# anonymousauthors001/SGS-GNN

Measured on AMD Instinct MI355X. Metric: sampled edges/sec + training steps/sec, Reddit hybrid 20% sparsity, higher is better.
Workload: dtype f32

## Files before the change

### sgs-gnn_amd/csrc/gcn.hip

```cpp
#include "sgs_common.h"

namespace sgs {
size_t graph_sort_workspace_bytes(int64_t n, int64_t N);
size_t graph_src_sorted_workspace_bytes(int64_t n, int64_t N);
int graph_build_src_sorted(const int64_t* ei, int64_t n, int64_t N, int32_t* in_ptr, int32_t* in_src, int32_t* in_eid, int32_t* out_ptr,
                           int32_t* out_dst, int32_t* out_eid, int32_t* loop_eid, int32_t* unsorted_flag, void* ws, size_t ws_bytes,
                           hipStream_t stream);
int graph_build_by_sort(const int64_t* ei, int64_t n, int64_t N, int32_t* in_ptr, int32_t* in_src, int32_t* in_eid, int32_t* out_ptr,
                        int32_t* out_dst, int32_t* out_eid, int32_t* loop_eid, void* ws, size_t ws_bytes, hipStream_t stream);
}

namespace sgs {
namespace {

constexpr int kT = 256;
constexpr int kMaxLdsRow = 8192;

__global__ void __launch_bounds__(kT) count_degrees(const int64_t* __restrict__ ei, int64_t n_edges, int* __restrict__ cnt_in,
                                                   int* __restrict__ cnt_out, int* __restrict__ loop_eid) {
    const int64_t e = static_cast<int64_t>(blockIdx.x) * kT + threadIdx.x;
    if (e >= n_edges) return;
    const int s = static_cast<int>(ei[e]), d = static_cast<int>(ei[n_edges + e]);
    atomicAdd(&cnt_in[d], 1);
    atomicAdd(&cnt_out[s], 1);
// ... 292 lines not shown
            cptr[row] = w;
            if (row == N - 1) cptr[N] = w + cnt[row];
        }
    } else {
        w = (out ? out_ptr : in_ptr)[row];
    }
    int loop = -1;
    const int b = pptr[row], e = pptr[row + 1];
    int pe_c = 0, col_c = 0;
    if (e > b) { const int kc = min(b + lane, e - 1); pe_c = peid[kc]; col_c = pcol[kc]; }
    for (int k0 = b; k0 < e; k0 += 64) {
        const int k = k0 + lane;
        const int kn = min(k + 64, e - 1);
        const int pe_n = peid[kn], col_n = pcol[kn];
        const bool m_c = mask_at<BITS>(mask, pe_c);
        const bool sel = k < e && m_c;
        const int ne = sel ? pos[pe_c] : 0;
        const int col = col_c;
        pe_c = pe_n; col_c = col_n;
        const unsigned long long bal = __ballot(sel);
        if (sel) {
            const int o = w + __popcll(bal & ((1ull << lane) - 1ull));
            ccol[o] = col;
            ceid[o] = ne;
        }
        if (!out) {
            const unsigned long long lb = __ballot(sel && col == static_cast<int>(row));
            if (lb) loop = __shfl(ne, 63 - __clzll(lb), 64);
        }
        w += __popcll(bal);
    }
    if (!out && lane == 0) loop_eid[row] = loop;
}
template <bool BITS, bool SCAN = false>
__global__ void __launch_bounds__(kT) filter_fill(const int* __restrict__ pin_ptr, const int* __restrict__ pin_src, const int* __restrict__ pin_eid,
                                                 const int* __restrict__ pout_ptr, const int* __restrict__ pout_dst,
                                                 const int* __restrict__ pout_eid, int64_t N, const uint8_t* __restrict__ mask,
                                                 const int* __restrict__ pos, int* __restrict__ in_ptr, int* __restrict__ in_src,
                                                 int* __restrict__ in_eid, int* __restrict__ out_ptr, int* __restrict__ out_dst,
                                                 int* __restrict__ out_eid, int* __restrict__ loop_eid, const int* __restrict__ cnt_in = nullptr,
                                                 const int* __restrict__ cnt_out = nullptr) {
    filter_fill_body<BITS, SCAN>(2 * N, pin_ptr, pin_src, pin_eid, pout_ptr, pout_dst, pout_eid, N, mask, pos, in_ptr, in_src, in_eid, out_ptr,
                                 out_dst, out_eid, loop_eid, cnt_in, cnt_out);
}

__device__ __forceinline__ void norm_deg_body(const float* __restrict__ w, int64_t N, const int* __restrict__ in_ptr,
                                              const int* __restrict__ in_src, const int* __restrict__ in_eid,
                                              const int* __restrict__ loop_eid, float* __restrict__ dis,
                                              float* __restrict__ loopw) {
    const int lane = threadIdx.x & 63;
    const int64_t i = (static_cast<int64_t>(blockIdx.x) * kT + threadIdx.x) >> 6;
    if (i >= N) return;
    const int b = in_ptr[i], e = in_ptr[i + 1];
    float acc = 0.f;
    for (int k = b + lane; k < e; k += 64) {
        if (in_src[k] != static_cast<int>(i)) acc += w ? w[in_eid[k]] : 1.0f;
    }
    acc = wave_sum_all(acc);
    const int le = loop_eid[i];
    const float lw = (le >= 0 && w) ? w[le] : 1.0f;
    const float deg = lw + acc;
    float di = 1.0f / sqrtf(deg);
    if (isinf(di)) di = 0.f;
    if (lane == 0) { dis[i] = di; loopw[i] = lw; }
}
__global__ void __launch_bounds__(kT) norm_deg(const float* __restrict__ w, int64_t N, const int* __restrict__ in_ptr,
                                              const int* __restrict__ in_src, const int* __restrict__ in_eid,
                                              const int* __restrict__ loop_eid, float* __restrict__ dis,
                                              float* __restrict__ loopw) {
    norm_deg_body(w, N, in_ptr, in_src, in_eid, loop_eid, dis, loopw);
}

__global__ void __launch_bounds__(kT) deg_partial(const float* __restrict__ w, int64_t N, const int* __restrict__ in_ptr,
                                                 const int* __restrict__ in_src, const int* __restrict__ in_eid,
                                                 float* __restrict__ degpart) {
    const int lane = threadIdx.x & 63;
    const int64_t i = (static_cast<int64_t>(blockIdx.x) * kT + threadIdx.x) >> 6;
    if (i >= N) return;
    float acc = 0.f;
    for (int k = in_ptr[i] + lane; k < in_ptr[i + 1]; k += 64)
        if (in_src[k] != static_cast<int>(i)) acc += w ? w[in_eid[k]] : 1.0f;
    acc = wave_sum_all(acc);
    if (lane == 0) degpart[i] = acc;
}
__global__ void __launch_bounds__(kT) dis_from_degree(const float* __restrict__ degsum, int64_t N, float* __restrict__ dis,
                                                     float* __restrict__ loopw) {
    const int64_t i = static_cast<int64_t>(blockIdx.x) * kT + threadIdx.x;
    if (i >= N) return;
    float di = 1.0f / sqrtf(1.0f + degsum[i]);
    if (isinf(di)) di = 0.f;
    dis[i] = di;
    loopw[i] = 1.0f;
}
__global__ void __launch_bounds__(kT) bias_act(const float* __restrict__ X, const float* __restrict__ bias, int64_t N, int64_t D, int act,
                                              float drop_scale, uint32_t drop_thresh, uint64_t seed, uint32_t site,
                                              const uint64_t* __restrict__ epoch, float* __restrict__ Y, int64_t row_offset) {
    seed = fold_epoch(seed, epoch);
    const int64_t idx = static_cast<int64_t>(blockIdx.x) * kT + threadIdx.x;
    if (idx >= N * D) return;
    const int64_t i = idx / D;
    const uint32_t c = static_cast<uint32_t>(idx - i * D);
    float y = X[idx];
    if (bias) y += bias[c];
    if (act != SGS_ACT_NONE) y = fmaxf(y, 0.f);
    if (act == SGS_ACT_RELU_DROPOUT) y = dropout_keep_at(seed, site, static_cast<uint64_t>(row_offset + i), c, drop_thresh) ? y * drop_scale : 0.f;
    Y[idx] = y;
}

__global__ void __launch_bounds__(kT) mean_weights(int64_t N, const int* __restrict__ in_ptr, const int* __restrict__ out_ptr,
                                                  const int* __restrict__ out_dst, float* __restrict__ what_in,
                                                  float* __restrict__ what_out) {
    const int lane = threadIdx.x & 63;
// ... 23 lines not shown
    logit[e] = prob * scale;
}

__device__ __forceinline__ void norm_weights_body(int64_t nrows, const float* __restrict__ w, int64_t N, int64_t n_edges,
                                                  const int* __restrict__ in_ptr, const int* __restrict__ in_src,
                                                  const int* __restrict__ in_eid, const int* __restrict__ out_ptr,
                                                  const int* __restrict__ out_dst, const int* __restrict__ out_eid,
                                                  const float* __restrict__ dis, const float* __restrict__ loopw,
                                                  float* __restrict__ what_in, float* __restrict__ what_out,
                                                  float* __restrict__ what_loop) {
    const int lane = threadIdx.x & 63;
    const int64_t r = (static_cast<int64_t>(blockIdx.x) * kT + threadIdx.x) >> 6;
    if (r >= nrows) return;
    const bool out = r >= N;
    const int i = static_cast<int>(out ? r - N : r);
    const float di = dis[i];
    if (!out) {
        const int b = in_ptr[i], e = in_ptr[i + 1];
        for (int k = b + lane; k < e; k += 64) {
            const int s = in_src[k];
            const float we = w ? w[in_eid[k]] : 1.0f;
            what_in[k] = (s == i) ? 0.f : (dis[s] * we) * di;
        }
        if (lane == 0) what_loop[i] = (di * loopw[i]) * di;
    } else {
        const int b = out_ptr[i], e = out_ptr[i + 1];
        for (int k = b + lane; k < e; k += 64) {
            const int t = out_dst[k];
            const float we = w ? w[out_eid[k]] : 1.0f;
            what_out[k] = (t == i) ? 0.f : (di * we) * dis[t];
        }
    }
}
__global__ void __launch_bounds__(kT) norm_weights(const float* __restrict__ w, int64_t N, int64_t n_edges,
                                                  const int* __restrict__ in_ptr, const int* __restrict__ in_src,
                                                  const int* __restrict__ in_eid, const int* __restrict__ out_ptr,
                                                  const int* __restrict__ out_dst, const int* __restrict__ out_eid,
                                                  const float* __restrict__ dis, const float* __restrict__ loopw,
                                                  float* __restrict__ what_in, float* __restrict__ what_out,
                                                  float* __restrict__ what_loop) {
    norm_weights_body(2 * N, w, N, n_edges, in_ptr, in_src, in_eid, out_ptr, out_dst, out_eid, dis, loopw, what_in, what_out, what_loop);
}

__global__ void __launch_bounds__(kT) norm_bwd_node(const float* __restrict__ w, const float* __restrict__ gw,
                                                   const float* __restrict__ gloop, int64_t N, const int* __restrict__ in_ptr,
                                                   const int* __restrict__ in_src, const int* __restrict__ in_eid,
                                                   const int* __restrict__ out_ptr, const int* __restrict__ out_dst,
                                                   const int* __restrict__ out_eid, const float* __restrict__ dis,
                                                   const float* __restrict__ loopw, float* __restrict__ Hn,
                                                   const float* __restrict__ gw2 = nullptr, const float* __restrict__ gloop2 = nullptr) {
    const int lane = threadIdx.x & 63;
    const int64_t t = (static_cast<int64_t>(blockIdx.x) * kT + threadIdx.x) >> 6;
    if (t >= N) return;
    float acc = 0.f;
    auto side = [&](const int* __restrict__ ptr, const int* __restrict__ col, const int* __restrict__ eid) {
        const int b = ptr[t], e_ = ptr[t + 1];
        for (int k0 = b; k0 < e_; k0 += 64) {
            const int k = k0 + lane, kc = min(k, e_ - 1);
            const int s = col[kc], e = eid[kc];
            const float ge = gw2 ? gw[e] + gw2[e] : gw[e];
            const float v = ge * w[e] * dis[s];
            if (k < e_ && s != static_cast<int>(t)) acc += v;
        }
    };
    side(in_ptr, in_src, in_eid);
    side(out_ptr, out_dst, out_eid);
    acc = wave_sum_all(acc);
    if (lane == 0) {
        const float a = dis[t];
        const float gl = gloop2 ? gloop[t] + gloop2[t] : gloop[t];
        const float G = acc + 2.0f * gl * loopw[t] * a;
        Hn[t] = -0.5f * a * a * a * G;
    }
}

__global__ void __launch_bounds__(kT) norm_bwd_edge(const float* __restrict__ gw, const float* __restrict__ gloop,
                                                   const int64_t* __restrict__ ei, int64_t n_edges,
                                                   const int* __restrict__ loop_eid, const float* __restrict__ dis,
                                                   const float* __restrict__ Hn, float* __restrict__ dw,
                                                   const float* __restrict__ gw2 = nullptr, const float* __restrict__ gloop2 = nullptr,
                                                   const float* __restrict__ dw_add = nullptr) {
    const int64_t e = static_cast<int64_t>(blockIdx.x) * kT + threadIdx.x;
    if (e >= n_edges) return;
    const int s = static_cast<int>(ei[e]), t = static_cast<int>(ei[n_edges + e]);
    float g;
    if (s != t) g = (gw2 ? gw[e] + gw2[e] : gw[e]) * dis[s] * dis[t] + Hn[t];
    else g = (gloop2 ? gloop[s] + gloop2[s] : gloop[s]) * dis[s] * dis[s] + Hn[s];
    dw[e] = dw_add ? g + dw_add[e] : g;
}

template <int VEC> struct VecT;
template <> struct VecT<1> { using type = float; };
template <> struct VecT<4> { using type = float4; };

__device__ __forceinline__ void fma_vec(float& a, float w, float x) { a = fmaf(w, x, a); }
__device__ __forceinline__ void fma_vec(float4& a, float w, const float4& x) {
    a.x = fmaf(w, x.x, a.x); a.y = fmaf(w, x.y, a.y); a.z = fmaf(w, x.z, a.z); a.w = fmaf(w, x.w, a.w);
}
__device__ __forceinline__ float4 zero4() { return make_float4(0.f, 0.f, 0.f, 0.f); }

__global__ void __launch_bounds__(kT) edge_reverse(const int64_t* __restrict__ ei, int64_t n, const int* __restrict__ out_ptr,
                                                  const int* __restrict__ out_dst, const int* __restrict__ out_eid, int* __restrict__ rev) {
    const int64_t e = static_cast<int64_t>(blockIdx.x) * kT + threadIdx.x;
    if (e >= n) return;
    const int s = static_cast<int>(ei[e]), d = static_cast<int>(ei[n + e]);
    int lo = out_ptr[d], hi = out_ptr[d + 1];
    const int end = hi;
    while (lo < hi) {
        const int mid = (lo + hi) >> 1;
        if (out_dst[mid] < s) lo = mid + 1; else hi = mid;
    }
    rev[e] = (lo < end && out_dst[lo] == s) ? out_eid[lo] : -1;
}
__global__ void __launch_bounds__(kT) edge_mate(const int* __restrict__ rev, int64_t n, int* __restrict__ mate) {
    const int64_t e = static_cast<int64_t>(blockIdx.x) * kT + threadIdx.x;
    if (e >= n) return;
    const int m = rev[e];
    mate[e] = (m >= 0 && m != e && rev[m] == static_cast<int>(e)) ? m : -1;
}

template <int VEC, int LPR>
__device__ __forceinline__ void spmm_csr_body(const float* __restrict__ X, int64_t N, int64_t D, const int* __restrict__ ptr,
                                              const int* __restrict__ col, const float* __restrict__ val,
                                              const float* __restrict__ diag, const float* __restrict__ bias, int act,
// ... 297 lines not shown
        const float d0 = wave_sum_all(dot(col[k]));
        if (lane == 0) g[eid[k]] = d0;
    }
    if (wave == 0 && gdiag) {
        const float d0 = wave_sum_all(dot(i));
        if (lane == 0) gdiag[i] = d0;
    }
}

__global__ void __launch_bounds__(kT) act_bwd(const float* __restrict__ dY, const float* __restrict__ Y, int64_t n, int act,
                                             float drop_scale, float* __restrict__ dZ) {
    const int64_t i = static_cast<int64_t>(blockIdx.x) * kT + threadIdx.x;
    if (i >= n) return;
    float g = dY[i];
    if (act != SGS_ACT_NONE) g = (Y[i] > 0.f) ? (act == SGS_ACT_RELU_DROPOUT ? g * drop_scale : g) : 0.f;
    dZ[i] = g;
}

constexpr int kColRows = 256;
inline int colsum_rows(int64_t N) { return N >= 16384 ? kColRows : (N >= 4096 ? 128 : 32); }
__global__ void __launch_bounds__(kT) colsum_partial(const float* __restrict__ A, int64_t N, int64_t D, int rows, float* __restrict__ part) {
    __shared__ float red[4][64];
    const int c = blockIdx.x * 64 + (threadIdx.x & 63);
    const int rgrp = threadIdx.x >> 6;
    const int64_t r0 = static_cast<int64_t>(blockIdx.y) * rows;
    const int64_t r1 = (r0 + rows < N) ? r0 + rows : N;
    float acc = 0.f;
    if (c < D)
        for (int64_t r = r0 + rgrp; r < r1; r += 4) acc += A[r * D + c];
    red[rgrp][threadIdx.x & 63] = acc;
    __syncthreads();
    if (rgrp == 0 && c < D)
        part[static_cast<int64_t>(blockIdx.y) * D + c] = (red[0][threadIdx.x] + red[1][threadIdx.x]) + (red[2][threadIdx.x] + red[3][threadIdx.x]);
}
template <int RG>
__global__ void __launch_bounds__(RG * 64) colsum_final(const float* __restrict__ part, int64_t nchunk, int64_t D, float* __restrict__ out) {
    __shared__ float red[RG][64];
    const int c = blockIdx.x * 64 + (threadIdx.x & 63);
    const int rgrp = threadIdx.x >> 6;
    float acc = 0.f;
    if (c < D)
        for (int64_t r = rgrp; r < nchunk; r += RG) acc += part[r * D + c];
    red[rgrp][threadIdx.x & 63] = acc;
    __syncthreads();
    if (rgrp == 0 && c < D) {
        float s = 0.f;
#pragma unroll
        for (int g = 0; g < RG; g += 4) s += (red[g][threadIdx.x] + red[g + 1][threadIdx.x]) + (red[g + 2][threadIdx.x] + red[g + 3][threadIdx.x]);
        out[c] = s;
    }
}

constexpr int kColSmallRows = 2048;
template <bool ACT>
__device__ __forceinline__ void colsum_small_body(const float* __restrict__ A, const float* __restrict__ Y, int64_t N, int64_t D, int act,
                                                  float drop_scale, float* __restrict__ dZ, float* __restrict__ out, int64_t blk) {
    __shared__ float red[64][17];
    const int cl = threadIdx.x & 15, rl = threadIdx.x >> 4;
    const int64_t c = blk * 16 + cl;
    float acc = 0.f;
    if (c < D) {
#pragma unroll 16
        for (int64_t r = rl; r < N; r += 64) {
            float g = A[r * D + c];
            if (ACT) {
                if (act != SGS_ACT_NONE) g = (Y[r * D + c] > 0.f) ? (act == SGS_ACT_RELU_DROPOUT ? g * drop_scale : g) : 0.f;
                dZ[r * D + c] = g;
            }
            acc += g;
        }
    }
    red[rl][cl] = acc;
    __syncthreads();
#pragma unroll
    for (int h = 32; h >= 1; h >>= 1) {
        if (rl < h) red[rl][cl] += red[rl + h][cl];
        __syncthreads();
    }
    if (rl == 0 && c < D && out) out[c] = red[0][cl];
}
template <bool ACT>
__global__ void __launch_bounds__(1024) colsum_small(const float* __restrict__ A, const float* __restrict__ Y, int64_t N, int64_t D, int act,
                                                    float drop_scale, float* __restrict__ dZ, float* __restrict__ out) {
    colsum_small_body<ACT>(A, Y, N, D, act, drop_scale, dZ, out, blockIdx.x);
}

template <bool ACT>
__device__ __forceinline__ void colsum_small_v4_body(const float* __restrict__ A, const float* __restrict__ Y, int64_t N, int64_t D, int act,
                                                     float drop_scale, float* __restrict__ dZ, float* __restrict__ out, int64_t blk) {
    __shared__ float4 red[256][4];
    const int cg = threadIdx.x & 3, rl = threadIdx.x >> 2;
    const int64_t c = blk * 16 + 4 * cg;
    float4 acc = make_float4(0.f, 0.f, 0.f, 0.f);
    if (c < D) {
#pragma unroll 8
        for (int64_t r = rl; r < N; r += 256) {
            float4 g = *reinterpret_cast<const float4*>(A + r * D + c);
            if (ACT) {
                if (act != SGS_ACT_NONE) {
                    const float4 y = *reinterpret_cast<const float4*>(Y + r * D + c);
                    const float sc = act == SGS_ACT_RELU_DROPOUT ? drop_scale : 1.f;
                    g.x = y.x > 0.f ? g.x * sc : 0.f; g.y = y.y > 0.f ? g.y * sc : 0.f;
                    g.z = y.z > 0.f ? g.z * sc : 0.f; g.w = y.w > 0.f ? g.w * sc : 0.f;
                }
                *reinterpret_cast<float4*>(dZ + r * D + c) = g;
            }
            acc.x += g.x; acc.y += g.y; acc.z += g.z; acc.w += g.w;
        }
    }
    red[rl][cg] = acc;
    __syncthreads();
#pragma unroll
    for (int h = 128; h >= 1; h >>= 1) {
        if (rl < h) {
            const float4 o = red[rl + h][cg];
            float4 m = red[rl][cg];
            m.x += o.x; m.y += o.y; m.z += o.z; m.w += o.w;
            red[rl][cg] = m;
        }
        __syncthreads();
    }
    if (rl == 0 && c < D && out) *reinterpret_cast<float4*>(out + c) = red[0][cg];
}
template <bool ACT>
__global__ void __launch_bounds__(1024) colsum_small_v4(const float* __restrict__ A, const float* __restrict__ Y, int64_t N, int64_t D, int act,
                                                       float drop_scale, float* __restrict__ dZ, float* __restrict__ out) {
    colsum_small_v4_body<ACT>(A, Y, N, D, act, drop_scale, dZ, out, blockIdx.x);
}

constexpr int64_t kVecSumMax = int64_t(1) << 20;
__global__ void __launch_bounds__(1024) vecsum_small(const float* __restrict__ A, int64_t N, float* __restrict__ out) {
    __shared__ float red[16];
    float a0 = 0.f, a1 = 0.f, a2 = 0.f, a3 = 0.f;
    int64_t i = threadIdx.x;
    for (; i + 3 * 1024 < N; i += 4 * 1024) { a0 += A[i]; a1 += A[i + 1024]; a2 += A[i + 2048]; a3 += A[i + 3072]; }
    for (; i < N; i += 1024) a0 += A[i];
    const float r = block_sum((a0 + a1) + (a2 + a3), red);
    if (threadIdx.x == 0) out[0] = r;
}


__global__ void __launch_bounds__(kT) multi_filter_count(const int* __restrict__ pin_ptr, const int* __restrict__ pin_eid, int64_t N, int64_t E,
                                                        const uint8_t* __restrict__ mask, const int64_t* __restrict__ sampled_eid, int64_t q,
                                                        int64_t n_row_blocks, int* __restrict__ cnt, int* __restrict__ pos) {
    const int64_t d = blockIdx.y;
    filter_count_scatter_body<false>(pin_ptr, pin_eid, nullptr, nullptr, N, mask + d * E, sampled_eid + d * q, q, n_row_blocks, cnt + d * (N + 1),
                                     nullptr, pos + d * E, N);
}
__global__ void __launch_bounds__(1024) multi_scan_counts(const int* __restrict__ cnt, int64_t N, int* __restrict__ in_ptr, int* __restrict__ cur) {
    const int64_t d = blockIdx.y;
    scan_counts_body(cnt + d * (N + 1), N, in_ptr + d * (N + 1), cur + d * (N + 1));
}
template <bool SCAN>
__global__ void __launch_bounds__(kT) multi_filter_fill(const int* __restrict__ pin_ptr, const int* __restrict__ pin_src, const int* __restrict__ pin_eid,
                                                       int64_t N, int64_t E, int64_t q, const uint8_t* __restrict__ mask, const int* __restrict__ pos,
                                                       int* __restrict__ in_ptr, int* __restrict__ in_src, int* __restrict__ in_eid,
                                                       int* __restrict__ loop_eid, const int* __restrict__ cnt) {
    const int64_t d = blockIdx.y;
    filter_fill_body<false, SCAN>(N, pin_ptr, pin_src, pin_eid, nullptr, nullptr, nullptr, N, mask + d * E, pos + d * E, in_ptr + d * (N + 1),
// ... 996 lines not shown
```

### sgs-gnn_amd/csrc/gemm_tn.hip

```cpp
#include "sgs_common.h"

namespace sgs {
namespace {

using f32x16 = __attribute__((ext_vector_type(16))) float;
constexpr int kUnroll = 8;

__global__ void __launch_bounds__(64) gemm_tn_tile(const float* __restrict__ A, const float* __restrict__ B, int64_t K, int M, int N,
                                                  int ksplit, float* __restrict__ slab) {
    const int lane = threadIdx.x, kh = lane >> 5, l31 = lane & 31;
    const int ti = blockIdx.x, tj = blockIdx.y, s = blockIdx.z;
    const int i = ti * 32 + l31, j = tj * 32 + l31;
    const bool iok = i < M, jok = j < N;
    const int64_t per = ((K + ksplit - 1) / ksplit + 1) & ~int64_t(1);
    const int64_t k0 = s * per, k1 = (k0 + per < K) ? k0 + per : K;
    f32x16 acc;
#pragma unroll
    for (int r = 0; r < 16; ++r) acc[r] = 0.f;
    int64_t k = k0;
    for (; k + 2 * kUnroll <= k1; k += 2 * kUnroll) {
        float a[kUnroll], b[kUnroll];
#pragma unroll
        for (int u = 0; u < kUnroll; ++u) {
            const int64_t kk = k + 2 * u + kh;
// ... 58 lines not shown
#pragma unroll
    for (int q = 0; q < RPW; ++q) {
        const int r = s * RPW + q;
        float sum = 0.f;
#pragma unroll
        for (int z = 0; z < NW; ++z) sum += red[z][r][lane];
        const int row = ti * 32 + (r & 3) + 8 * (r >> 2) + 4 * kh;
        if (row < M) C[static_cast<int64_t>(row) * ldc + j] = sum;
    }
}

template <int NW>
__global__ void __launch_bounds__(64 * NW) gemm_tn_wg(const float* __restrict__ A, const float* __restrict__ B, int64_t K, int M, int N,
                                                     float* __restrict__ C, int64_t ldc) {
    gemm_tn_wg_tile<NW>(A, B, K, M, N, C, ldc, blockIdx.x, blockIdx.y);
}

constexpr int kGroupMax = 8;
struct GemmTnDesc {
    const float* A;
    const float* B;
    float* C;
    int64_t K, ldc;
    int M, N;
    int first_tile, tiles_i;
};
struct GemmTnGroupArgs {
    GemmTnDesc d[kGroupMax];
    int count;
};

template <int NW>
__global__ void __launch_bounds__(64 * NW) gemm_tn_wg_group(GemmTnGroupArgs a) {
    const int t = static_cast<int>(blockIdx.x);
    int pi = 0;
    while (pi + 1 < a.count && t >= a.d[pi + 1].first_tile) ++pi;
    const GemmTnDesc& d = a.d[pi];
    const int local = t - d.first_tile;
    const int tj = local / d.tiles_i, ti = local - tj * d.tiles_i;
    gemm_tn_wg_tile<NW>(d.A, d.B, d.K, d.M, d.N, d.C, d.ldc, ti, tj);
}

__global__ void __launch_bounds__(256) gemm_tn_reduce(const float* __restrict__ slab, int64_t mn, int ksplit, float* __restrict__ C,
                                                      const float* __restrict__ cpart = nullptr, int M = 0, float* __restrict__ colsum = nullptr,
                                                      int N = 0, int64_t ldc = 0, const float* __restrict__ rowscale = nullptr,
                                                      float scale = 1.f, const float* __restrict__ dzpart = nullptr, int nz = 0,
                                                      float* __restrict__ dzsum = nullptr, float* __restrict__ Craw = nullptr,
                                                      float* __restrict__ csraw = nullptr, int csplit = 0) {
    const int64_t i = static_cast<int64_t>(blockIdx.x) * 256 + threadIdx.x;
    if (i >= mn) {
        const int64_t c = i - mn;
        if (dzsum && c == M) {
            float acc = 0.f;
            for (int z = 0; z < nz; ++z) acc += dzpart[z];
            dzsum[0] = acc;
        }
        if (colsum && c < M) {
            float acc = 0.f;
            const int ncs = csplit > 0 ? csplit : ksplit;
            if (csplit > 0) {
                float a8[8] = {0.f, 0.f, 0.f, 0.f, 0.f, 0.f, 0.f, 0.f};
                int s = 0;
                for (; s + 8 <= ncs; s += 8) {
                    float v[8];
#pragma unroll
                    for (int j = 0; j < 8; ++j) v[j] = cpart[static_cast<int64_t>(s + j) * M + c];
#pragma unroll
                    for (int j = 0; j < 8; ++j) a8[j] += v[j];
                }
                for (; s < ncs; ++s) a8[0] += cpart[static_cast<int64_t>(s) * M + c];
                acc = ((a8[0] + a8[1]) + (a8[2] + a8[3])) + ((a8[4] + a8[5]) + (a8[6] + a8[7]));
            } else
            for (int s = 0; s < ncs; ++s) acc += cpart[static_cast<int64_t>(s) * M + c];
            if (csraw) csraw[c] = acc;
            colsum[c] = rowscale ? acc * (rowscale[c] * scale) : acc;
        }
        return;
    }
    float acc = 0.f;
    if (csplit > 0) {
        float a8[8] = {0.f, 0.f, 0.f, 0.f, 0.f, 0.f, 0.f, 0.f};
        int s = 0;
        for (; s + 8 <= ksplit; s += 8) {
            float v[8];
#pragma unroll
            for (int j = 0; j < 8; ++j) v[j] = slab[static_cast<int64_t>(s + j) * mn + i];
#pragma unroll
            for (int j = 0; j < 8; ++j) a8[j] += v[j];
        }
        for (; s < ksplit; ++s) a8[0] += slab[static_cast<int64_t>(s) * mn + i];
        acc = ((a8[0] + a8[1]) + (a8[2] + a8[3])) + ((a8[4] + a8[5]) + (a8[6] + a8[7]));
    } else
    for (int s = 0; s < ksplit; ++s) acc += slab[static_cast<int64_t>(s) * mn + i];
    if (Craw) Craw[i] = acc;
    if (rowscale) acc *= rowscale[i / N] * scale;
    if (ldc > 0 && ldc != N) C[(i / N) * ldc + (i % N)] = acc;
    else C[i] = acc;
}

constexpr int kTallK = 8192;
constexpr int kTallU = 8;

__global__ void __launch_bounds__(64) gemm_tn_tall_tile(const float* __restrict__ A, const float* __restrict__ B, int64_t K, int M, int N,
                                                       int ksplit, float* __restrict__ slab, float* __restrict__ cpart) {
    const int lane = threadIdx.x, kh = lane >> 5, l31 = lane & 31;
    const int m0 = blockIdx.x * 128, n0 = blockIdx.y * 64, s = blockIdx.z;
    const int ia = m0 + 4 * l31, jb = n0 + 2 * l31;
    const bool aok = ia < M, bok = jb < N;
    const int64_t per = ((K + ksplit - 1) / ksplit + 1) & ~int64_t(1);
    const int64_t k0 = s * per, k1 = (k0 + per < K) ? k0 + per : K;
    f32x16 acc[4][2];
#pragma unroll
    for (int t = 0; t < 4; ++t)
#pragma unroll
        for (int u = 0; u < 2; ++u)
#pragma unroll
            for (int r = 0; r < 16; ++r) acc[t][u][r] = 0.f;
    const float4 z4 = make_float4(0.f, 0.f, 0.f, 0.f);
    const float2 z2 = make_float2(0.f, 0.f);
    const bool want_cs = cpart != nullptr && blockIdx.y == 0;
    float cs[4] = {0.f, 0.f, 0.f, 0.f};
    auto load = [&](int64_t k, float4 (&a)[kTallU], float2 (&b)[kTallU]) {
#pragma unroll
        for (int u = 0; u < kTallU; ++u) {
            const int64_t kk = k + 2 * u + kh;
            const bool in = kk < k1;
            a[u] = (aok && in) ? *reinterpret_cast<const float4*>(A + kk * M + ia) : z4;
            b[u] = (bok && in) ? *reinterpret_cast<const float2*>(B + kk * N + jb) : z2;
        }
    };
    auto mma = [&](const float4 (&a)[kTallU], const float2 (&b)[kTallU]) {
#pragma unroll
        for (int u = 0; u < kTallU; ++u) {
            const float av[4] = {a[u].x, a[u].y, a[u].z, a[u].w};
            const float bv[2] = {b[u].x, b[u].y};
// ... 862 lines not shown
```

### sgs-gnn_amd/csrc/optim.hip

```cpp
#include "sgs_common.h"

namespace sgs {
namespace {

constexpr int kAT = 256;
constexpr int kAChunk = 2048;
constexpr int kAMax = 24;

struct AdamDesc {
    float* p;
    const float* g;
    float* m;
    float* v;
    int64_t n;
    float* step;
    const float* gate;
};
struct AdamArgs {
    AdamDesc d[kAMax];
    int chunk_end[kAMax];
    int n_tensors;
    float lr, beta1, beta2, eps, weight_decay;
    int maximize;
    unsigned int* ticket;
};

__global__ void __launch_bounds__(kAT) adam_group(AdamArgs a) {
    __shared__ unsigned int s_last;
    int ti = 0;
    while (static_cast<int>(blockIdx.x) >= a.chunk_end[ti]) ++ti;
    const int chunk = static_cast<int>(blockIdx.x) - (ti ? a.chunk_end[ti - 1] : 0);
    const AdamDesc d = a.d[ti];
    const bool open = d.gate == nullptr || d.gate[0] != 0.f;
    const float t = d.step[0] + 1.0f;
    const double bc1 = 1.0 - exp(static_cast<double>(t) * log(static_cast<double>(a.beta1)));
    const double bc2 = 1.0 - exp(static_cast<double>(t) * log(static_cast<double>(a.beta2)));
    const float step_size = static_cast<float>(static_cast<double>(a.lr) / bc1);
    const float inv_sqrt_bc2 = static_cast<float>(1.0 / sqrt(bc2));
    const float beta1 = a.beta1, beta2 = a.beta2, eps = a.eps, wd = a.weight_decay;
    const int64_t base = static_cast<int64_t>(chunk) * kAChunk;
#pragma unroll
    for (int it = 0; it < kAChunk / kAT; ++it) {
        const int64_t i = base + static_cast<int64_t>(it) * kAT + threadIdx.x;
        if (open && i < d.n) {
            float g = d.g[i];
            if (a.maximize) g = -g;
            const float p = d.p[i];
            if (wd != 0.f) g = fmaf(wd, p, g);
            float m = d.m[i], v = d.v[i];
            m = m + (g - m) * (1.0f - beta1);
            v = beta2 * v + (1.0f - beta2) * g * g;
            const float denom = sqrtf(v) * inv_sqrt_bc2 + eps;
            d.m[i] = m;
            d.v[i] = v;
            d.p[i] = p - step_size * (m / denom);
        }
    }
    __syncthreads();
    if (threadIdx.x == 0) s_last = (atomicAdd(a.ticket, 1u) == gridDim.x - 1) ? 1u : 0u;
    __syncthreads();
    if (s_last) {
        if (static_cast<int>(threadIdx.x) < a.n_tensors) {
            const AdamDesc& dd = a.d[threadIdx.x];
            if (dd.gate == nullptr || dd.gate[0] != 0.f) dd.step[0] += 1.0f;
        }
        if (threadIdx.x == 0) __hip_atomic_store(a.ticket, 0u, __ATOMIC_RELAXED, __HIP_MEMORY_SCOPE_AGENT);
    }
}

constexpr int kAMax2 = 16;
struct AdamState {
    float* m;
    float* v;
    float* step;
    const float* gate;
    float lr, beta1, beta2, eps, wd;
    int maximize;
};
struct AdamDesc2 {
    float* p;
    const float* g;
    int64_t n;
    AdamState s[2];
    int n_states;
};
struct AdamArgs2 {
    AdamDesc2 d[kAMax2];
    int chunk_end[kAMax2];
    int n_tensors;
    unsigned int* ticket;
    float* loss_sum;
    const float* loss;
    unsigned long long* epoch;
};

__global__ void __launch_bounds__(kAT) adam_multi(AdamArgs2 a) {
    __shared__ unsigned int s_last;
    int ti = 0;
    while (static_cast<int>(blockIdx.x) >= a.chunk_end[ti]) ++ti;
    const int chunk = static_cast<int>(blockIdx.x) - (ti ? a.chunk_end[ti - 1] : 0);
    const AdamDesc2& d = a.d[ti];
    bool open[2];
    float step_size[2], inv_sqrt_bc2[2];
#pragma unroll
    for (int q = 0; q < 2; ++q) {
        open[q] = q < d.n_states && (d.s[q].gate == nullptr || d.s[q].gate[0] != 0.f);
        step_size[q] = 0.f;
        inv_sqrt_bc2[q] = 0.f;
        if (q < d.n_states) {
            const float t = d.s[q].step[0] + 1.0f;
            const double bc1 = 1.0 - exp(static_cast<double>(t) * log(static_cast<double>(d.s[q].beta1)));
            const double bc2 = 1.0 - exp(static_cast<double>(t) * log(static_cast<double>(d.s[q].beta2)));
            step_size[q] = static_cast<float>(static_cast<double>(d.s[q].lr) / bc1);
            inv_sqrt_bc2[q] = static_cast<float>(1.0 / sqrt(bc2));
        }
    }
    const int64_t base = static_cast<int64_t>(chunk) * kAChunk;
#pragma unroll
    for (int it = 0; it < kAChunk / kAT; ++it) {
        const int64_t i = base + static_cast<int64_t>(it) * kAT + threadIdx.x;
        if (i < d.n && (open[0] || open[1])) {
            const float g0 = d.g[i];
            float p = d.p[i];
#pragma unroll
            for (int q = 0; q < 2; ++q) {
                if (open[q]) {
                    const AdamState& st = d.s[q];
                    float g = st.maximize ? -g0 : g0;
                    if (st.wd != 0.f) g = fmaf(st.wd, p, g);
                    float m = st.m[i], v = st.v[i];
                    m = m + (g - m) * (1.0f - st.beta1);
                    v = st.beta2 * v + (1.0f - st.beta2) * g * g;
                    const float denom = sqrtf(v) * inv_sqrt_bc2[q] + st.eps;
                    st.m[i] = m;
                    st.v[i] = v;
                    p = p - step_size[q] * (m / denom);
                }
            }
            d.p[i] = p;
        }
    }
    __syncthreads();
    if (threadIdx.x == 0) s_last = (atomicAdd(a.ticket, 1u) == gridDim.x - 1) ? 1u : 0u;
    __syncthreads();
    if (s_last) {
        if (static_cast<int>(threadIdx.x) < 2 * a.n_tensors) {
            const AdamDesc2& dd = a.d[threadIdx.x >> 1];
            const int q = threadIdx.x & 1;
            if (q < dd.n_states && (dd.s[q].gate == nullptr || dd.s[q].gate[0] != 0.f)) {
                dd.s[q].step[0] += 1.0f;
            }
        }
        if (threadIdx.x == 64) {
            if (a.loss_sum && a.loss) a.loss_sum[0] += a.loss[0];
            if (a.epoch) a.epoch[0] += 1ull;
        }
        if (threadIdx.x == 0) __hip_atomic_store(a.ticket, 0u, __ATOMIC_RELAXED, __HIP_MEMORY_SCOPE_AGENT);
    }
}

}
}

using namespace sgs;

extern "C" {

int sgs_adam_max_tensors(void) { return kAMax; }

int sgs_adam_step(const int64_t* desc_host, int64_t n_tensors, float lr, float beta1, float beta2, float eps, float weight_decay,
                  int maximize, uint32_t* ticket, sgs_stream_t stream_) {
    hipStream_t stream = static_cast<hipStream_t>(stream_);
    SGS_REQUIRE(n_tensors >= 0 && n_tensors <= kAMax, SGS_EINVAL, "sgs_adam_step: at most %d tensors per call", kAMax);
    if (n_tensors == 0) return SGS_OK;
    SGS_REQUIRE(desc_host && ticket, SGS_EINVAL, "sgs_adam_step: null pointer");
    SGS_REQUIRE(beta1 >= 0.f && beta1 < 1.f && beta2 >= 0.f && beta2 < 1.f && eps >= 0.f, SGS_EINVAL, "sgs_adam_step: bad hyper-parameters");
    AdamArgs a{};
    int64_t total = 0;
    for (int i = 0; i < kAMax; ++i) {
        if (i < n_tensors) {
            const int64_t* w = desc_host + 7 * i;
            a.d[i].p = reinterpret_cast<float*>(w[0]);
            a.d[i].g = reinterpret_cast<const float*>(w[1]);
            a.d[i].m = reinterpret_cast<float*>(w[2]);
            a.d[i].v = reinterpret_cast<float*>(w[3]);
            a.d[i].n = w[4];
            a.d[i].step = reinterpret_cast<float*>(w[5]);
            a.d[i].gate = reinterpret_cast<const float*>(w[6]);
            SGS_REQUIRE(a.d[i].p && a.d[i].g && a.d[i].m && a.d[i].v && a.d[i].step && a.d[i].n >= 0, SGS_EINVAL,
                        "sgs_adam_step: bad descriptor %d", i);
            total += cdiv(a.d[i].n, kAChunk);
        }
        a.chunk_end[i] = static_cast<int>(total);
    }
// ... 59 lines not shown
```

Measured before the change: 112.6 million.

## Batch loads ahead of compute in norm, colsum, reduction and Adam kernels

Several kernels are changed to issue their global loads before any dependent arithmetic. norm_deg and norm_bwd_node hoist per-node loads and load unconditionally so the reads can overlap. The colsum activation paths load R rows into registers before computing, and the split-K reduction in gemm_tn gains 32-wide unrolled batches separated by sched_barrier. The Adam kernels are rewritten into a templated chunk routine that uses float4 loads when pointers are aligned, loads all state up front, and specialises on the number of optimizer states. The cost is higher register pressure and extra loads of data that is then discarded.

```diff
diff --git a/sgs-gnn_amd/csrc/gcn.hip b/sgs-gnn_amd/csrc/gcn.hip
--- a/sgs-gnn_amd/csrc/gcn.hip
+++ b/sgs-gnn_amd/csrc/gcn.hip
@@ -368,12 +368,14 @@
     const int64_t i = (static_cast<int64_t>(blockIdx.x) * kT + threadIdx.x) >> 6;
     if (i >= N) return;
     const int b = in_ptr[i], e = in_ptr[i + 1];
+    const int le = loop_eid[i];
     float acc = 0.f;
     for (int k = b + lane; k < e; k += 64) {
-        if (in_src[k] != static_cast<int>(i)) acc += w ? w[in_eid[k]] : 1.0f;
+        const int s = in_src[k], id = (w ? in_eid : in_src)[k];
+        const float we = w ? w[id] : 1.0f;
+        acc += (s != static_cast<int>(i)) ? we : 0.f;
     }
     acc = wave_sum_all(acc);
-    const int le = loop_eid[i];
     const float lw = (le >= 0 && w) ? w[le] : 1.0f;
     const float deg = lw + acc;
     float di = 1.0f / sqrtf(deg);
@@ -503,24 +505,26 @@
     const int lane = threadIdx.x & 63;
     const int64_t t = (static_cast<int64_t>(blockIdx.x) * kT + threadIdx.x) >> 6;
     if (t >= N) return;
+    const int b_in = in_ptr[t], e_in = in_ptr[t + 1], b_out = out_ptr[t], e_out = out_ptr[t + 1];
+    const float a = dis[t], lw = loopw[t], gl1 = gloop[t], gl2 = (gloop2 ? gloop2 : gloop)[t];
+    const float* __restrict__ gwb = gw2 ? gw2 : gw;
     float acc = 0.f;
-    auto side = [&](const int* __restrict__ ptr, const int* __restrict__ col, const int* __restrict__ eid) {
-        const int b = ptr[t], e_ = ptr[t + 1];
+    auto side = [&](const int b, const int e_, const int* __restrict__ col, const int* __restrict__ eid) {
         for (int k0 = b; k0 < e_; k0 += 64) {
             const int k = k0 + lane, kc = min(k, e_ - 1);
             const int s = col[kc], e = eid[kc];
-            const float ge = gw2 ? gw[e] + gw2[e] : gw[e];
-            const float v = ge * w[e] * dis[s];
-            if (k < e_ && s != static_cast<int>(t)) acc += v;
+            const float g1 = gw[e], g2 = gwb[e], we = w[e], ds = dis[s];
+            const float ge = gw2 ? g1 + g2 : g1;
+            const float v = ge * we * ds;
+            acc += (k < e_ && s != static_cast<int>(t)) ? v : 0.f;
         }
     };
-    side(in_ptr, in_src, in_eid);
-    side(out_ptr, out_dst, out_eid);
+    side(b_in, e_in, in_src, in_eid);
+    side(b_out, e_out, out_dst, out_eid);
     acc = wave_sum_all(acc);
     if (lane == 0) {
-        const float a = dis[t];
-        const float gl = gloop2 ? gloop[t] + gloop2[t] : gloop[t];
-        const float G = acc + 2.0f * gl * loopw[t] * a;
+        const float gl = gloop2 ? gl1 + gl2 : gl1;
+        const float G = acc + 2.0f * gl * lw * a;
         Hn[t] = -0.5f * a * a * a * G;
     }
 }
@@ -924,6 +928,71 @@
 }
 
 constexpr int kColSmallRows = 2048;
+__device__ __forceinline__ float colsum_act_rows(const float* __restrict__ A, const float* __restrict__ Y, int64_t N, int64_t D, int act, float drop_scale,
+                                                 float* __restrict__ dZ, int64_t c, int rl) {
+    constexpr int R = 16;
+    float acc = 0.f;
+    for (int64_t r0 = rl; r0 - rl < N; r0 += 64 * R) {
+        float g[R], y[R];
+#pragma unroll
+        for (int k = 0; k < R; ++k) {
+            const int64_t r = r0 + 64 * k;
+            g[k] = A[(r < N ? r : N - 1) * D + c];
+        }
+        if (act != SGS_ACT_NONE) {
+#pragma unroll
+            for (int k = 0; k < R; ++k) {
+                const int64_t r = r0 + 64 * k;
+                y[k] = Y[(r < N ? r : N - 1) * D + c];
+            }
+#pragma unroll
+            for (int k = 0; k < R; ++k) g[k] = (y[k] > 0.f) ? (act == SGS_ACT_RELU_DROPOUT ? g[k] * drop_scale : g[k]) : 0.f;
+        }
+#pragma unroll
+        for (int k = 0; k < R; ++k) {
+            const int64_t r = r0 + 64 * k;
+            if (r < N) dZ[r * D + c] = g[k];
+        }
+#pragma unroll
+        for (int k = 0; k < R; ++k)
+            if (r0 + 64 * k < N) acc += g[k];
+    }
+    return acc;
+}
+template <int R>
+__device__ __forceinline__ float4 colsum_act_rows_v4(const float* __restrict__ A, const float* __restrict__ Y, int64_t N, int64_t D, int act,
+                                                     float drop_scale, float* __restrict__ dZ, int64_t c, int rl) {
+    float4 g[R], y[R];
+#pragma unroll
+    for (int k = 0; k < R; ++k) {
+        const int64_t r = rl + 256 * k;
+        g[k] = *reinterpret_cast<const float4*>(A + (r < N ? r : N - 1) * D + c);
+    }
+    if (act != SGS_ACT_NONE) {
+#pragma unroll
+        for (int k = 0; k < R; ++k) {
+            const int64_t r = rl + 256 * k;
+            y[k] = *reinterpret_cast<const float4*>(Y + (r < N ? r : N - 1) * D + c);
+        }
+        const float sc = act == SGS_ACT_RELU_DROPOUT ? drop_scale : 1.f;
+#pragma unroll
+        for (int k = 0; k < R; ++k) {
+            g[k].x = y[k].x > 0.f ? g[k].x * sc : 0.f; g[k].y = y[k].y > 0.f ? g[k].y * sc : 0.f;
+            g[k].z = y[k].z > 0.f ? g[k].z * sc : 0.f; g[k].w = y[k].w > 0.f ? g[k].w * sc : 0.f;
+        }
+    }
+#pragma unroll
+    for (int k = 0; k < R; ++k) {
+        const int64_t r = rl + 256 * k;
+        if (r < N) *reinterpret_cast<float4*>(dZ + r * D + c) = g[k];
+    }
+    float4 acc = make_float4(0.f, 0.f, 0.f, 0.f);
+#pragma unroll
+    for (int k = 0; k < R; ++k)
+        if (rl + 256 * k < N) { acc.x += g[k].x; acc.y += g[k].y; acc.z += g[k].z; acc.w += g[k].w; }
+    return acc;
+}
+
 template <bool ACT>
 __device__ __forceinline__ void colsum_small_body(const float* __restrict__ A, const float* __restrict__ Y, int64_t N, int64_t D, int act,
                                                   float drop_scale, float* __restrict__ dZ, float* __restrict__ out, int64_t blk) {
@@ -931,16 +1000,11 @@
     const int cl = threadIdx.x & 15, rl = threadIdx.x >> 4;
     const int64_t c = blk * 16 + cl;
     float acc = 0.f;
-    if (c < D) {
+    if (ACT) {
+        if (c < D) acc = colsum_act_rows(A, Y, N, D, act, drop_scale, dZ, c, rl);
+    } else if (c < D) {
 #pragma unroll 16
-        for (int64_t r = rl; r < N; r += 64) {
-            float g = A[r * D + c];
-            if (ACT) {
-                if (act != SGS_ACT_NONE) g = (Y[r * D + c] > 0.f) ? (act == SGS_ACT_RELU_DROPOUT ? g * drop_scale : g) : 0.f;
-                dZ[r * D + c] = g;
-            }
-            acc += g;
-        }
+        for (int64_t r = rl; r < N; r += 64) acc += A[r * D + c];
     }
     red[rl][cl] = acc;
     __syncthreads();
@@ -964,19 +1028,15 @@
     const int cg = threadIdx.x & 3, rl = threadIdx.x >> 2;
     const int64_t c = blk * 16 + 4 * cg;
     float4 acc = make_float4(0.f, 0.f, 0.f, 0.f);
-    if (c < D) {
+    if (ACT) {
+        if (c < D) {
+            if (N <= 4 * 256) acc = colsum_act_rows_v4<4>(A, Y, N, D, act, drop_scale, dZ, c, rl);
+            else              acc = colsum_act_rows_v4<kColSmallRows / 256>(A, Y, N, D, act, drop_scale, dZ, c, rl);
+        }
+    } else if (c < D) {
 #pragma unroll 8
         for (int64_t r = rl; r < N; r += 256) {
-            float4 g = *reinterpret_cast<const float4*>(A + r * D + c);
-            if (ACT) {
-                if (act != SGS_ACT_NONE) {
-                    const float4 y = *reinterpret_cast<const float4*>(Y + r * D + c);
-                    const float sc = act == SGS_ACT_RELU_DROPOUT ? drop_scale : 1.f;
-                    g.x = y.x > 0.f ? g.x * sc : 0.f; g.y = y.y > 0.f ? g.y * sc : 0.f;
-                    g.z = y.z > 0.f ? g.z * sc : 0.f; g.w = y.w > 0.f ? g.w * sc : 0.f;
-                }
-                *reinterpret_cast<float4*>(dZ + r * D + c) = g;
-            }
+            const float4 g = *reinterpret_cast<const float4*>(A + r * D + c);
             acc.x += g.x; acc.y += g.y; acc.z += g.z; acc.w += g.w;
         }
     }
diff --git a/sgs-gnn_amd/csrc/gemm_tn.hip b/sgs-gnn_amd/csrc/gemm_tn.hip
--- a/sgs-gnn_amd/csrc/gemm_tn.hip
+++ b/sgs-gnn_amd/csrc/gemm_tn.hip
@@ -134,7 +134,15 @@
         const int64_t c = i - mn;
         if (dzsum && c == M) {
             float acc = 0.f;
-            for (int z = 0; z < nz; ++z) acc += dzpart[z];
+            int z = 0;
+            for (; z + 16 <= nz; z += 16) {
+                float v[16];
+#pragma unroll
+                for (int j = 0; j < 16; ++j) v[j] = dzpart[z + j];
+#pragma unroll
+                for (int j = 0; j < 16; ++j) acc += v[j];
+            }
+            for (; z < nz; ++z) acc += dzpart[z];
             dzsum[0] = acc;
         }
         if (colsum && c < M) {
@@ -143,6 +151,14 @@
             if (csplit > 0) {
                 float a8[8] = {0.f, 0.f, 0.f, 0.f, 0.f, 0.f, 0.f, 0.f};
                 int s = 0;
+                for (; s + 32 <= ncs; s += 32) {
+                    float v[32];
+#pragma unroll
+                    for (int j = 0; j < 32; ++j) v[j] = cpart[static_cast<int64_t>(s + j) * M + c];
+                    __builtin_amdgcn_sched_barrier(0);
+#pragma unroll
+                    for (int j = 0; j < 32; ++j) a8[j & 7] += v[j];
+                }
                 for (; s + 8 <= ncs; s += 8) {
                     float v[8];
 #pragma unroll
@@ -163,6 +179,14 @@
     if (csplit > 0) {
         float a8[8] = {0.f, 0.f, 0.f, 0.f, 0.f, 0.f, 0.f, 0.f};
         int s = 0;
+        for (; s + 32 <= ksplit; s += 32) {
+            float v[32];
+#pragma unroll
+            for (int j = 0; j < 32; ++j) v[j] = slab[static_cast<int64_t>(s + j) * mn + i];
+            __builtin_amdgcn_sched_barrier(0);
+#pragma unroll
+            for (int j = 0; j < 32; ++j) a8[j & 7] += v[j];
+        }
         for (; s + 8 <= ksplit; s += 8) {
             float v[8];
 #pragma unroll
diff --git a/sgs-gnn_amd/csrc/optim.hip b/sgs-gnn_amd/csrc/optim.hip
--- a/sgs-gnn_amd/csrc/optim.hip
+++ b/sgs-gnn_amd/csrc/optim.hip
@@ -25,37 +25,129 @@
     unsigned int* ticket;
 };
 
+template <int NS>
+struct AdamRun {
+    float* p;
+    const float* g;
+    int64_t n;
+    float* m[NS];
+    float* v[NS];
+    const float* step[NS];
+    const float* gate[NS];
+    float lr[NS], beta1[NS], beta2[NS], eps[NS], wd[NS];
+    bool maximize[NS];
+};
+
+template <int W> struct AdamWord;
+template <> struct AdamWord<1> { using T = float; };
+template <> struct AdamWord<4> { using T = float4; };
+template <int W>
+__device__ __forceinline__ void adam_ld(const float* q, float (&x)[W]) {
+    const typename AdamWord<W>::T t = *reinterpret_cast<const typename AdamWord<W>::T*>(q);
+    __builtin_memcpy(x, &t, sizeof(t));
+}
+template <int W>
+__device__ __forceinline__ void adam_st(float* q, const float (&x)[W]) {
+    typename AdamWord<W>::T t;
+    __builtin_memcpy(&t, x, sizeof(t));
+    *reinterpret_cast<typename AdamWord<W>::T*>(q) = t;
+}
+
+template <int NS, int W>
+__device__ __forceinline__ void adam_chunk(const AdamRun<NS>& r, int64_t base) {
+    constexpr int IT = kAChunk / (kAT * W);
+    const int left = static_cast<int>(r.n - base < kAChunk ? r.n - base : kAChunk);
+    float t[NS], gw[NS];
+#pragma unroll
+    for (int q = 0; q < NS; ++q) {
+        t[q] = r.step[q][0];
+        gw[q] = (r.gate[q] ? r.gate[q] : r.step[q])[0];
+    }
+    const float* gb = r.g + base;
+    float* pb = r.p + base;
+    int off[IT], at[IT];
+    float g0[IT][W], p[IT][W], m[NS][IT][W], v[NS][IT][W];
+#pragma unroll
+    for (int it = 0; it < IT; ++it) {
+        off[it] = (it * kAT + static_cast<int>(threadIdx.x)) * W;
+        at[it] = W > 1 ? off[it] : (off[it] < left ? off[it] : left - 1);
+        adam_ld<W>(gb + at[it], g0[it]);
+        adam_ld<W>(pb + at[it], p[it]);
+    }
+#pragma unroll
+    for (int q = 0; q < NS; ++q)
+#pragma unroll
+        for (int it = 0; it < IT; ++it) {
+            adam_ld<W>(r.m[q] + base + at[it], m[q][it]);
+            adam_ld<W>(r.v[q] + base + at[it], v[q][it]);
+        }
+    __builtin_amdgcn_sched_barrier(0);
+    bool open[NS];
+    float step_size[NS], inv_sqrt_bc2[NS];
+#pragma unroll
+    for (int q = 0; q < NS; ++q) {
+        open[q] = r.gate[q] == nullptr || gw[q] != 0.f;
+        const float tt = t[q] + 1.0f;
+        const double bc1 = 1.0 - exp(static_cast<double>(tt) * log(static_cast<double>(r.beta1[q])));
+        const double bc2 = 1.0 - exp(static_cast<double>(tt) * log(static_cast<double>(r.beta2[q])));
+        step_size[q] = static_cast<float>(static_cast<double>(r.lr[q]) / bc1);
+        inv_sqrt_bc2[q] = static_cast<float>(1.0 / sqrt(bc2));
+    }
+#pragma unroll
+    for (int q = 0; q < NS; ++q) {
+        if (!open[q]) continue;
+        const float beta1 = r.beta1[q], beta2 = r.beta2[q], eps = r.eps[q], wd = r.wd[q];
+#pragma unroll
+        for (int it = 0; it < IT; ++it)
+#pragma unroll
+            for (int k = 0; k < W; ++k) {
+                float g = r.maximize[q] ? -g0[it][k] : g0[it][k];
+                if (wd != 0.f) g = fmaf(wd, p[it][k], g);
+                float mm = m[q][it][k], vv = v[q][it][k];
+                mm = mm + (g - mm) * (1.0f - beta1);
+                vv = beta2 * vv + (1.0f - beta2) * g * g;
+                const float denom = sqrtf(vv) * inv_sqrt_bc2[q] + eps;
+                m[q][it][k] = mm;
+                v[q][it][k] = vv;
+                p[it][k] = p[it][k] - step_size[q] * (mm / denom);
+            }
+    }
+    bool any = false;
+#pragma unroll
+    for (int q = 0; q < NS; ++q) any = any || open[q];
+#pragma unroll
+    for (int it = 0; it < IT; ++it) {
+        if (off[it] >= left) continue;
+#pragma unroll
+        for (int q = 0; q < NS; ++q)
+            if (open[q]) {
+                adam_st<W>(r.m[q] + base + off[it], m[q][it]);
+                adam_st<W>(r.v[q] + base + off[it], v[q][it]);
+            }
+        if (any) adam_st<W>(pb + off[it], p[it]);
+    }
+}
+
+template <int NS>
+__device__ __forceinline__ void adam_run(const AdamRun<NS>& r, int chunk) {
+    const int64_t base = static_cast<int64_t>(chunk) * kAChunk;
+    uintptr_t bits = reinterpret_cast<uintptr_t>(r.p) | reinterpret_cast<uintptr_t>(r.g);
+#pragma unroll
+    for (int q = 0; q < NS; ++q) bits |= reinterpret_cast<uintptr_t>(r.m[q]) | reinterpret_cast<uintptr_t>(r.v[q]);
+    if ((bits & 15) == 0 && base + kAChunk <= r.n) adam_chunk<NS, 4>(r, base);
+    else adam_chunk<NS, 1>(r, base);
+}
+
 __global__ void __launch_bounds__(kAT) adam_group(AdamArgs a) {
     __shared__ unsigned int s_last;
     int ti = 0;
     while (static_cast<int>(blockIdx.x) >= a.chunk_end[ti]) ++ti;
     const int chunk = static_cast<int>(blockIdx.x) - (ti ? a.chunk_end[ti - 1] : 0);
     const AdamDesc d = a.d[ti];
-    const bool open = d.gate == nullptr || d.gate[0] != 0.f;
-    const float t = d.step[0] + 1.0f;
-    const double bc1 = 1.0 - exp(static_cast<double>(t) * log(static_cast<double>(a.beta1)));
-    const double bc2 = 1.0 - exp(static_cast<double>(t) * log(static_cast<double>(a.beta2)));
-    const float step_size = static_cast<float>(static_cast<double>(a.lr) / bc1);
-    const float inv_sqrt_bc2 = static_cast<float>(1.0 / sqrt(bc2));
-    const float beta1 = a.beta1, beta2 = a.beta2, eps = a.eps, wd = a.weight_decay;
-    const int64_t base = static_cast<int64_t>(chunk) * kAChunk;
-#pragma unroll
-    for (int it = 0; it < kAChunk / kAT; ++it) {
-        const int64_t i = base + static_cast<int64_t>(it) * kAT + threadIdx.x;
-        if (open && i < d.n) {
-            float g = d.g[i];
-            if (a.maximize) g = -g;
-            const float p = d.p[i];
-            if (wd != 0.f) g = fmaf(wd, p, g);
-            float m = d.m[i], v = d.v[i];
-            m = m + (g - m) * (1.0f - beta1);
-            v = beta2 * v + (1.0f - beta2) * g * g;
-            const float denom = sqrtf(v) * inv_sqrt_bc2 + eps;
-            d.m[i] = m;
-            d.v[i] = v;
-            d.p[i] = p - step_size * (m / denom);
-        }
-    }
+    AdamRun<1> r;
+    r.p = d.p; r.g = d.g; r.n = d.n; r.m[0] = d.m; r.v[0] = d.v; r.step[0] = d.step; r.gate[0] = d.gate;
+    r.lr[0] = a.lr; r.beta1[0] = a.beta1; r.beta2[0] = a.beta2; r.eps[0] = a.eps; r.wd[0] = a.weight_decay; r.maximize[0] = a.maximize != 0;
+    adam_run<1>(r, chunk);
     __syncthreads();
     if (threadIdx.x == 0) s_last = (atomicAdd(a.ticket, 1u) == gridDim.x - 1) ? 1u : 0u;
     __syncthreads();
@@ -94,52 +186,27 @@
     unsigned long long* epoch;
 };
 
+template <int NS>
+__device__ __forceinline__ void adam_multi_run(const AdamDesc2& d, int chunk) {
+    AdamRun<NS> r;
+    r.p = d.p; r.g = d.g; r.n = d.n;
+#pragma unroll
+    for (int q = 0; q < NS; ++q) {
+        const AdamState& st = d.s[q];
+        r.m[q] = st.m; r.v[q] = st.v; r.step[q] = st.step; r.gate[q] = st.gate;
+        r.lr[q] = st.lr; r.beta1[q] = st.beta1; r.beta2[q] = st.beta2; r.eps[q] = st.eps; r.wd[q] = st.wd; r.maximize[q] = st.maximize != 0;
+    }
+    adam_run<NS>(r, chunk);
+}
+
 __global__ void __launch_bounds__(kAT) adam_multi(AdamArgs2 a) {
     __shared__ unsigned int s_last;
     int ti = 0;
     while (static_cast<int>(blockIdx.x) >= a.chunk_end[ti]) ++ti;
     const int chunk = static_cast<int>(blockIdx.x) - (ti ? a.chunk_end[ti - 1] : 0);
     const AdamDesc2& d = a.d[ti];
-    bool open[2];
-    float step_size[2], inv_sqrt_bc2[2];
-#pragma unroll
-    for (int q = 0; q < 2; ++q) {
-        open[q] = q < d.n_states && (d.s[q].gate == nullptr || d.s[q].gate[0] != 0.f);
-        step_size[q] = 0.f;
-        inv_sqrt_bc2[q] = 0.f;
-        if (q < d.n_states) {
-            const float t = d.s[q].step[0] + 1.0f;
-            const double bc1 = 1.0 - exp(static_cast<double>(t) * log(static_cast<double>(d.s[q].beta1)));
-            const double bc2 = 1.0 - exp(static_cast<double>(t) * log(static_cast<double>(d.s[q].beta2)));
-            step_size[q] = static_cast<float>(static_cast<double>(d.s[q].lr) / bc1);
-            inv_sqrt_bc2[q] = static_cast<float>(1.0 / sqrt(bc2));
-        }
-    }
-    const int64_t base = static_cast<int64_t>(chunk) * kAChunk;
-#pragma unroll
-    for (int it = 0; it < kAChunk / kAT; ++it) {
-        const int64_t i = base + static_cast<int64_t>(it) * kAT + threadIdx.x;
-        if (i < d.n && (open[0] || open[1])) {
-            const float g0 = d.g[i];
-            float p = d.p[i];
-#pragma unroll
-            for (int q = 0; q < 2; ++q) {
-                if (open[q]) {
-                    const AdamState& st = d.s[q];
-                    float g = st.maximize ? -g0 : g0;
-                    if (st.wd != 0.f) g = fmaf(st.wd, p, g);
-                    float m = st.m[i], v = st.v[i];
-                    m = m + (g - m) * (1.0f - st.beta1);
-                    v = st.beta2 * v + (1.0f - st.beta2) * g * g;
-                    const float denom = sqrtf(v) * inv_sqrt_bc2[q] + st.eps;
-                    st.m[i] = m;
-                    st.v[i] = v;
-                    p = p - step_size[q] * (m / denom);
-                }
-            }
-            d.p[i] = p;
-        }
-    }
+    if (d.n_states > 1) adam_multi_run<2>(d, chunk);
+    else adam_multi_run<1>(d, chunk);
     __syncthreads();
     if (threadIdx.x == 0) s_last = (atomicAdd(a.ticket, 1u) == gridDim.x - 1) ? 1u : 0u;
     __syncthreads();
```

Result: faster. 114.6 million, median of 6 (+1.8%).
